# hcherkaoui/pybold

Measured on AMD Instinct MI355X. Metric: voxel-iterations/sec, higher is better.
Workload: dtype f16x2-split operands (22 bit), f32 accumulate, f64 iterate

## Files before the change

### include/pybold_hip.h

```cpp
#ifndef PYBOLD_HIP_H
#define PYBOLD_HIP_H

#include <stdint.h>

#ifdef __cplusplus
extern "C" {
#endif

#define PB_OK 0
#define PB_ERR_INVALID (-1)
#define PB_ERR_HIP (-2)

#define PB_FLAG_FORCE_GENERIC 1u
#define PB_FLAG_FORCE_FAST 2u
#define PB_FLAG_NO_PAIR 4u
#define PB_FLAG_FORCE_PAIR 8u
#define PB_FLAG_FORCE_WIDE 16u
#define PB_FLAG_DIRECT_FIR 64u
#define PB_FLAG_ONE_STREAM 128u
#define PB_FLAG_COLD_START 256u
#define PB_FLAG_NO_CERT 512u
#define PB_FLAG_CERT_NO_RESOLVE 2048u
#define PB_FLAG_FORCE_MFMA 16384u
#define PB_FLAG_NO_RHO_GUARD 32768u
#define PB_FLAG_FORCE_MFMA2 65536u
#define PB_FLAG_NO_MFMA 8192u
#define PB_FLAG_FORCE_CERT 1024u
#define PB_FLAG_NO_PARTITION 4096u
#define PB_FLAG_ONLY_DENSE 131072u
#define PB_FLAG_ONLY_SPARSE 262144u
#define PB_FLAG_NO_ILL_GUARD 524288u
#define PB_FLAG_PP_SPLIT 1048576u
#define PB_FLAG_LONG_HRF 2097152u
#define PB_FLAG_ONE_LAUNCH 32u

#define PB_STOP_NONE 0
#define PB_STOP_LOOPS 1
#define PB_STOP_WINDOW 2

int pb_version(void);

int pb_init(void);

const char* pb_last_error(void);

int pb_fista_has_fast_path(int N, int K);

int pb_fista_which_kernel(int N, int K, int P, int with_cost_trace, int stop_mode, int wind);

int pb_fista_plan(int N, int K, int P, int stop_mode, int wind, int* n_main, int* main_form,
                  int* tail_form);
int pb_fista_plan_ex(int N, int K, int P, int stop_mode, int wind, unsigned flags, int* n_main,
                     int* main_form, int* tail_form);

int pb_fista_solve(const float* y_dev, int64_t ldy, int y_rep,
                   double* w_dev, int64_t ldw, int P, int N,
                   const double* taps_host, const double* taps_dev, int K,
                   double step, double lbda, const double* lbda_dev,
                   const double* betas_dev, int n_iter,
                   float* J_dev, int64_t ldj,
                   int stop_mode, double tol, int wind, int32_t* n_done_dev,
                   unsigned flags, void* stream);

int64_t pb_fista_work_len(int P, int y_rep);
#define PB_CAND_COUNT 10
int pb_fista_list_plan(int kind, int n, int n_max, int has_pair, int has_wide, int one_stream, int has_mfma2,
                       int beside_chunks, int32_t* ranges, int32_t* bounds);
int pb_fista_solve_ex(const float* y_dev, int64_t ldy, int y_rep,
                      double* w_dev, int64_t ldw, int P, int N,
                      const double* taps_host, const double* taps_dev, int K,
                      double step, double lbda, const double* lbda_dev,
                      const double* betas_dev, int n_iter,
                      float* J_dev, int64_t ldj,
                      int stop_mode, double tol, int wind, int32_t* n_done_dev,
                      unsigned flags, void* stream,
                      const double* lmax_dev, double dense_ratio, int32_t* work_dev, int64_t work_len);

#define PB_PATH_DENSE_RATIO 0.19
#define PB_PATH_DENSE_RATIO_LONG 0.22
#define PB_PATH_DENSE_RATIO_LONGER 0.26
int64_t pb_fista_path_work_len(int P);
int pb_fista_solve_path(const float* y_dev, int64_t ldy, int y_rep, double* w_dev, int64_t ldw, int P, int N,
                        const double* taps_host, const double* taps_dev, int K, double step,
                        const double* lbda_dev, const double* lmax_dev, double dense_ratio,
                        const double* betas_dev, int n_iter, int32_t* n_done_dev, int32_t* work_dev,
                        int64_t work_len, unsigned flags, void* stream);

int pb_fista_outputs(const double* w_dev, int64_t ldw, int P, int N,
                     const double* taps_dev, int K,
                     double* z_dev, int64_t ldz, double* x_dev, int64_t ldx,
                     void* stream);

int pb_fista_stats(const double* w_dev, int64_t ldw, const float* y_dev, int64_t ldy,
                   int y_rep, int P, int N, const double* taps_dev, int K,
                   double* r2_dev, double* l1_dev, void* stream);

int pb_integ_op(const double* x_dev, int64_t ldx, double* out_dev, int64_t ldo,
                int V, int N, void* stream);
int pb_integ_adj(const double* x_dev, int64_t ldx, double* out_dev, int64_t ldo,
                 int V, int N, void* stream);
// ... 172 lines not shown
```

### pybold_amd/_lib.py

```python
import ctypes
import os

_HERE = os.path.dirname(os.path.abspath(__file__))
LIB_PATH = os.environ.get("PYBOLD_HIP_LIB") or os.path.join(_HERE, "libpybold_hip.so")

PB_FLAG_FORCE_GENERIC = 1
PB_FLAG_FORCE_FAST = 2
PB_FLAG_NO_PAIR = 4
PB_FLAG_FORCE_PAIR = 8
PB_FLAG_FORCE_WIDE = 16
PB_FLAG_ONE_LAUNCH = 32
PB_FLAG_DIRECT_FIR = 64
PB_FLAG_ONE_STREAM = 128
PB_FLAG_COLD_START = 256
PB_FLAG_NO_CERT = 512
PB_FLAG_FORCE_CERT = 1024
PB_FLAG_CERT_NO_RESOLVE = 2048
PB_FLAG_NO_PARTITION = 4096
PB_FLAG_NO_MFMA = 8192
PB_FLAG_FORCE_MFMA = 16384
PB_FLAG_NO_RHO_GUARD = 32768
PB_FLAG_FORCE_MFMA2 = 65536
PB_FLAG_ONLY_DENSE = 131072
PB_FLAG_ONLY_SPARSE = 262144
PB_FLAG_NO_ILL_GUARD = 524288
PB_FLAG_PP_SPLIT = 1048576
PB_FLAG_LONG_HRF = 2097152
PB_PATH_DENSE_RATIO = 0.19
PB_STOP_NONE = 0
PB_STOP_LOOPS = 1
PB_STOP_WINDOW = 2

_c_int = ctypes.c_int
_c_i64 = ctypes.c_int64
_c_dbl = ctypes.c_double
_ptr = ctypes.c_void_p

SIGNATURES = {
    "pb_version": (_c_int, []),
    "pb_init": (_c_int, []),
    "pb_last_error": (ctypes.c_char_p, []),
    "pb_fista_has_fast_path": (_c_int, [_c_int, _c_int]),
    "pb_fista_which_kernel": (_c_int, [_c_int, _c_int, _c_int, _c_int, _c_int, _c_int]),
    "pb_fista_plan": (_c_int, [_c_int, _c_int, _c_int, _c_int, _c_int, _ptr, _ptr, _ptr]),
    "pb_fista_plan_ex": (_c_int, [_c_int, _c_int, _c_int, _c_int, _c_int, ctypes.c_uint, _ptr, _ptr, _ptr]),
    "pb_fista_solve": (_c_int, [
        _ptr, _c_i64, _c_int,
        _ptr, _c_i64, _c_int, _c_int,
        _ptr, _ptr, _c_int,
        _c_dbl, _c_dbl, _ptr,
        _ptr, _c_int,
        _ptr, _c_i64,
        _c_int, _c_dbl, _c_int, _ptr,
        ctypes.c_uint, _ptr]),
    "pb_fista_work_len": (_c_i64, [_c_int, _c_int]),
    "pb_fista_list_plan": (_c_int, [_c_int, _c_int, _c_int, _c_int, _c_int, _c_int, _c_int, _c_int, _ptr, _ptr]),
    "pb_fista_solve_ex": (_c_int, [
        _ptr, _c_i64, _c_int,
        _ptr, _c_i64, _c_int, _c_int,
        _ptr, _ptr, _c_int,
        _c_dbl, _c_dbl, _ptr,
        _ptr, _c_int,
        _ptr, _c_i64,
        _c_int, _c_dbl, _c_int, _ptr,
        ctypes.c_uint, _ptr,
        _ptr, _c_dbl, _ptr, _c_i64]),
    "pb_fista_solve_backtrack_d": (_c_int, [
        _ptr, _c_i64, _c_int, _ptr, _c_i64, _c_int, _c_int,
        _ptr, _c_int, _c_dbl, _c_dbl, _c_int,
        _c_dbl, _ptr, _ptr, _c_int,
        _ptr, _ptr, _ptr, ctypes.c_uint, _ptr]),
    "pb_fista_path_work_len": (_c_i64, [_c_int]),
    "pb_fista_solve_path": (_c_int, [
        _ptr, _c_i64, _c_int,
        _ptr, _c_i64, _c_int, _c_int,
        _ptr, _ptr, _c_int,
        _c_dbl, _ptr, _ptr, _c_dbl,
        _ptr, _c_int,
        _ptr, _ptr, _c_i64,
        ctypes.c_uint, _ptr]),
    "pb_fista_outputs": (_c_int, [_ptr, _c_i64, _c_int, _c_int, _ptr, _c_int,
                                  _ptr, _c_i64, _ptr, _c_i64, _ptr]),
    "pb_fista_stats": (_c_int, [_ptr, _c_i64, _ptr, _c_i64, _c_int, _c_int, _c_int, _ptr,
                                _c_int, _ptr, _ptr, _ptr]),
    "pb_integ_op": (_c_int, [_ptr, _c_i64, _ptr, _c_i64, _c_int, _c_int, _ptr]),
    "pb_integ_adj": (_c_int, [_ptr, _c_i64, _ptr, _c_i64, _c_int, _c_int, _ptr]),
    "pb_conv": (_c_int, [_ptr, _c_i64, _ptr, _c_i64, _c_int, _c_int, _c_int,
                         _ptr, _c_int, _ptr]),
    "pb_corr": (_c_int, [_ptr, _c_i64, _ptr, _c_i64, _c_int, _c_int, _c_int,
# ... 181 lines not shown
```

### pybold_amd/csrc/capi.hip

```cpp
#include "../../include/pybold_hip.h"

#include <cstdarg>
#include <cstdlib>
#include <cstdio>
#include <cmath>
#include <cstring>
#include <map>
#include <mutex>

#include "fista_fast.h"
#include "generic.h"
#include "launch_fast.h"
#include "fista_pair.h"
#include "fista_pair_ffa.h"
#include "fista_exact.h"
#include "fista_exact_split.h"
#include "fista_auto.h"
#include "fista_exact_pp.h"
#include "fista_exact_split_pp.h"
#include "blind.h"
#include "fista_mfma.h"
#include "fista_mfma2.h"
#include "fista_mfma4.h"
#include "path.h"
#include "dispatch.h"

namespace {

thread_local char g_err[512] = "";

int fail(int code, const char* fmt, ...) {
  va_list ap;
  va_start(ap, fmt);
  vsnprintf(g_err, sizeof(g_err), fmt, ap);
  va_end(ap);
  return code;
}

int check_launch(const char* what) {
  hipError_t e = hipGetLastError();
  if (e != hipSuccess) return fail(PB_ERR_HIP, "%s: %s", what, hipGetErrorString(e));
  g_err[0] = 0;
  return PB_OK;
}

constexpr int LDS_DOUBLES_MAX = 20000;
inline int64_t gen_lds_doubles(int N, int K, int stop_mode, int wind) {
  return 3 * (int64_t)N + K + 2 * pb::GEN_WAVES + (stop_mode == PB_STOP_WINDOW ? (int64_t)wind * N : 0);
}

constexpr int AUTO_LAUNCH_ITERS = 65536, AUTO_RESIDENT_WAVES = 2048;
inline int auto_outer_chunk(int V, int nb_sub_iter) {
  const int64_t rounds = ((int64_t)V + AUTO_RESIDENT_WAVES - 1) / AUTO_RESIDENT_WAVES;
  const int64_t per = (int64_t)(nb_sub_iter > 0 ? nb_sub_iter : 1) * (rounds > 0 ? rounds : 1);
// ... 648 lines not shown
    return run_partition(r, a, lf, user, taps_host, taps_dev, flags, dense_ratio, work_dev);
  if (r.path != PATH_GENERIC) return run_in_place(r, a, lf, user, flags);
  if (flags & PB_FLAG_FORCE_FAST)
    return fail(PB_ERR_INVALID, "pb_fista_solve: no register-resident kernel for N=%d K=%d stop=%d",
                N, K, stop_mode);
  if (!taps_dev) return fail(PB_ERR_INVALID, "pb_fista_solve: taps_dev required for the generic kernel");
  if (gen_lds_doubles(N, K, stop_mode, wind) > LDS_DOUBLES_MAX)
    return fail(PB_ERR_INVALID, "pb_fista_solve: N=%d K=%d wind=%d exceeds LDS", N, K, wind);
  launch_generic(a, taps_dev, K, wind, J_dev != nullptr, false, P, user);
  return check_launch("fista_generic_kernel");
}

int pb_fista_list_plan(int kind, int n, int n_max, int has_pair, int has_wide, int one_stream, int has_mfma2,
                       int beside_chunks, int32_t* ranges, int32_t* bounds) {
  if (kind < 1 || kind > 3 || n < 0 || n_max < n) return fail(PB_ERR_INVALID, "pb_fista_list_plan: bad argument");
  Piece pc[pb::MAX_PIECES];
  int npc = 0;
  const double slots = wave_slots();
  if (n > 0 && kind == 1) npc = pb::plan_pieces_mfma(n, has_pair != 0, has_wide != 0, false, one_stream != 0, has_mfma2 != 0, beside_chunks, slots, pc);
  else if (n > 0 && kind == 2) npc = pb::plan_pieces(n, has_pair != 0, has_wide != 0, false, one_stream != 0, slots, pc);
  else if (kind == 3 && n_max > 0)
    npc = pb::plan_partitioned(n, n_max, has_pair != 0, has_wide != 0, one_stream != 0, has_mfma2 != 0, beside_chunks, slots, pc);
  int32_t rg[2 * pb::CAND_COUNT];
  const int rc = pb::plan_to_candidates(pc, npc, rg);
  for (int c = 0; c < pb::CAND_COUNT; ++c) {
    if (ranges) { ranges[2 * c] = rg[2 * c]; ranges[2 * c + 1] = rg[2 * c + 1]; }
    if (bounds) bounds[c] = pb::cand_max_slots(c, n_max, slots);
  }
  if (rc != 0) return fail(PB_ERR_INVALID, "pb_fista_list_plan: a piece of the plan found its candidate launch taken (n=%d)", n);
  g_err[0] = 0;
  return PB_OK;
}

int64_t pb_fista_work_len(int P, int y_rep) {
  if (P < 0 || y_rep < 1) return 0;
  return work_layout(P, (P + y_rep - 1) / y_rep).total;
}

int pb_fista_solve_ex(const float* y_dev, int64_t ldy, int y_rep, double* w_dev, int64_t ldw, int P,
                      int N, const double* taps_host, const double* taps_dev, int K, double step,
                      double lbda, const double* lbda_dev, const double* betas_dev, int n_iter, float* J_dev,
                      int64_t ldj, int stop_mode, double tol, int wind, int32_t* n_done_dev,
                      unsigned flags, void* stream, const double* lmax_dev, double dense_ratio,
                      int32_t* work_dev, int64_t work_len) {
  return solve_impl(y_dev, ldy, y_rep, w_dev, ldw, P, N, taps_host, taps_dev, K, step, lbda, lbda_dev, betas_dev, n_iter,
                    J_dev, ldj, stop_mode, tol, wind, n_done_dev, flags, stream, lmax_dev, dense_ratio, work_dev, work_len);
}

int pb_fista_solve(const float* y_dev, int64_t ldy, int y_rep, double* w_dev, int64_t ldw, int P,
                   int N, const double* taps_host, const double* taps_dev, int K, double step,
                   double lbda,
                   const double* lbda_dev, const double* betas_dev, int n_iter, float* J_dev,
                   int64_t ldj, int stop_mode, double tol, int wind, int32_t* n_done_dev,
                   unsigned flags, void* stream) {
  int32_t* work = nullptr;
  int64_t len = 0;
  if (P >= PART_MIN_P && N <= 1280 && n_done_dev && !(flags & PB_FLAG_NO_PARTITION) && !stream_is_capturing((hipStream_t)stream))
    work = own_workspace(stream, work_layout(P, (P + (y_rep > 0 ? y_rep : 1) - 1) / (y_rep > 0 ? y_rep : 1)).total, &len);
  return solve_impl(y_dev, ldy, y_rep, w_dev, ldw, P, N, taps_host, taps_dev, K, step, lbda, lbda_dev, betas_dev, n_iter,
                    J_dev, ldj, stop_mode, tol, wind, n_done_dev, flags, stream, nullptr, 0.0, work, len);
}

namespace {
int long_hrf_entry(const char* name, int N, int K, int stop_mode, int wind, unsigned flags, const ExactLongEntry** le) {
  if (flags & (PB_FLAG_FORCE_GENERIC | PB_FLAG_FORCE_FAST | PB_FLAG_PP_SPLIT))
    return fail(PB_ERR_INVALID, "%s: PB_FLAG_LONG_HRF names the 48-tap register form; it excludes PB_FLAG_FORCE_GENERIC, PB_FLAG_FORCE_FAST and PB_FLAG_PP_SPLIT", name);
// ... 763 lines not shown
```

### pybold_amd/csrc/dispatch.h

```cpp
#pragma once
#include "../../include/pybold_hip.h"
#include "fista_fast.h"
#include "launch_fast.h"
#include "fista_pair.h"
#include "fista_pair_ffa.h"
#include "fista_exact.h"
#include "fista_exact_split.h"
#include "fista_auto.h"
#include "fista_auto_split.h"
#include "fista_exact_pp.h"
#include "fista_exact_long.h"
#include "fista_exact_split_long.h"
#include "fista_mfma.h"
#include "fista_mfma2.h"
#include "fista_mfma4.h"
#include "path.h"

namespace {

typedef int (*fast_launch_fn)(const pb::FistaArgs&, const double* taps, int K, bool with_j,
                              int stop, hipStream_t);
typedef int (*fast_launch_pp_fn)(const pb::FistaArgs&, int stop, hipStream_t);
typedef int (*launch_fn)(const pb::FistaArgs&, const double* taps, int K, bool with_j, hipStream_t);
typedef int (*pair_cert_fn)(const pb::FistaArgs&, const double* taps, int K, hipStream_t);
typedef int (*pair_split_fn)(const pb::FistaArgs&, const double* taps, int K, bool with_j, bool cert, hipStream_t);

struct FastEntry {
  int S, KT;
  fast_launch_fn fn;
  fast_launch_pp_fn fn_pp;
  launch_fn fn_pair;
  launch_fn fn_pair_ffa;
  int (*fn_pair_dev)(const pb::FistaArgs&, hipStream_t);
  pair_cert_fn fn_pair_cert;
  pair_split_fn fn_pair_split;
};

}

namespace pb {
#define PB_FAST(S, KT)                                                                              \
  extern template int launch_fast<S, KT>(const FistaArgs&, const double*, int, bool, int, hipStream_t); \
  extern template int launch_fast_pp<S, KT>(const FistaArgs&, int, hipStream_t);            \
  extern template int launch_pair<S, KT>(const FistaArgs&, const double*, int, bool, hipStream_t); \
  extern template int launch_pair_ffa<S, KT>(const FistaArgs&, const double*, int, bool, hipStream_t); \
  extern template int launch_pair_ffa_dev<S, KT>(const FistaArgs&, hipStream_t);                  \
  extern template int launch_pair_ffa_cert<S, KT>(const FistaArgs&, const double*, int, hipStream_t); \
  extern template int launch_pair_ffa_split<S, KT>(const FistaArgs&, const double*, int, bool, bool, hipStream_t);
#include "fast_table.inc"
#undef PB_FAST
}

namespace pb {
#define PB_MFMA(NB) extern template int launch_mfma<NB>(const FistaArgs&, const double*, int, bool, hipStream_t);
PB_MFMA(5) PB_MFMA(6) PB_MFMA(7) PB_MFMA(8) PB_MFMA(9) PB_MFMA(10)
#undef PB_MFMA
}
namespace pb {
#define PB_MFMA2(A, B) extern template int launch_mfma2<A, B>(const FistaArgs&, const double*, int, bool, hipStream_t);
PB_MFMA2(2, 3) PB_MFMA2(3, 3) PB_MFMA2(3, 4) PB_MFMA2(4, 4) PB_MFMA2(4, 5) PB_MFMA2(5, 5) PB_MFMA2(5, 6) PB_MFMA2(6, 6)
PB_MFMA2(6, 7) PB_MFMA2(7, 7) PB_MFMA2(7, 8) PB_MFMA2(8, 8) PB_MFMA2(8, 9) PB_MFMA2(9, 9) PB_MFMA2(9, 10) PB_MFMA2(10, 10)
#undef PB_MFMA2
#define PB_MFMA4(A) extern template int launch_mfma4<A>(const FistaArgs&, const double*, int, bool, hipStream_t);
PB_MFMA4(6) PB_MFMA4(7) PB_MFMA4(8) PB_MFMA4(9) PB_MFMA4(10)
#undef PB_MFMA4
}
namespace {
launch_fn pick_mfma2(int N, int K, bool two_tiles_only) {
  static const launch_fn tab[] = {
      &pb::launch_mfma2<2, 3>, &pb::launch_mfma2<3, 3>, &pb::launch_mfma2<3, 4>, &pb::launch_mfma2<4, 4>,
      &pb::launch_mfma2<4, 5>, &pb::launch_mfma2<5, 5>, &pb::launch_mfma2<5, 6>, &pb::launch_mfma2<6, 6>,
      &pb::launch_mfma2<6, 7>, &pb::launch_mfma2<7, 7>, &pb::launch_mfma2<7, 8>, &pb::launch_mfma2<8, 8>,
      &pb::launch_mfma2<8, 9>, &pb::launch_mfma2<9, 9>, &pb::launch_mfma2<9, 10>, &pb::launch_mfma2<10, 10>};
  const int nb = (N + 31) / 32;
  if (K < 1 || K > 65 || nb < 5 || nb > 20) return nullptr;
  if (K > 33 && (two_tiles_only || N <= 224)) return nullptr;
  return tab[nb - 5];
}
launch_fn pick_mfma4(int N, int K, bool two_tiles_only) {
  static const launch_fn tab[] = {&pb::launch_mfma4<6>, &pb::launch_mfma4<7>, &pb::launch_mfma4<8>, &pb::launch_mfma4<9>,
                                  &pb::launch_mfma4<10>};
  if (K < 1 || K > 65 || (K > 33 && two_tiles_only) || N <= 640 || N > 1280) return nullptr;
  return tab[(N + 127) / 128 - 6];
}
constexpr int MFMA_K2 = 33, MFMA_K3 = 64;
constexpr int MFMA1_NMAX = 10 * pb::MFMA_SPAN;
launch_fn pick_mfma(int N, int K, bool stop_rule) {
  static const launch_fn tab[] = {&pb::launch_mfma<5>, &pb::launch_mfma<6>, &pb::launch_mfma<7>,
                                  &pb::launch_mfma<8>, &pb::launch_mfma<9>, &pb::launch_mfma<10>};
  const int nb = (N + pb::MFMA_SPAN - 1) / pb::MFMA_SPAN;
  if (K < 1 || K > MFMA_K3 || (K > MFMA_K2 && stop_rule) || N <= 128 || nb > 10) return nullptr;
  return tab[nb - 5];
}
}
namespace pb {
#define PB_WIDE(S, KT)                                                                            \
  extern template int launch_wide<S, KT>(const FistaArgs&, const double*, int, bool, int, hipStream_t); \
  extern template int launch_wide_pp<S, KT>(const FistaArgs&, int, hipStream_t);
#include "wide_table.inc"
#undef PB_WIDE
}
namespace {

typedef int (*wide_launch_fn)(const pb::FistaArgs&, const double* taps, int K, bool with_j, int stop,
                              hipStream_t);
struct WideEntry {
  int S, KT;
  wide_launch_fn fn;
  fast_launch_pp_fn fn_pp;
};
#define PB_WIDE(S, KT) {S, KT, &pb::launch_wide<S, KT>, &pb::launch_wide_pp<S, KT>},
const WideEntry kWide[] = {
#include "wide_table.inc"
};
#undef PB_WIDE

template <class Entry, size_t n>
const Entry* pick_cheapest(const Entry (&tab)[n], int N, int K, int per_lane) {
  const Entry* best = nullptr;
  const int s_need = (N + per_lane - 1) / per_lane;
  for (const Entry& e : tab) {
    if (e.S < s_need || e.KT < K) continue;
    if (!best || (int64_t)e.S * e.KT < (int64_t)best->S * best->KT) best = &e;
  }
  return best;
// ... 347 lines not shown
    r.cert = split_pair_cert;
    r.has_pair = r.se && (plain || split_pair_cert);
    return r;
  }
  const bool forced = (fl & PB_FLAG_FORCE_MFMA2) != 0;
  const bool forced_short = c.reported && forced && (plain || window6) && pick_mfma2(N, K, true);
  const launch_fn split = mfma4 ? mfma4 : ((mfma2 && ((forced && (!c.reported || long_shape || forced_short)) || long_call)) ? mfma2 : nullptr);
  if (split && (backup_ok || forced_short)) {
    r.path = PATH_SPLIT_LONG;
    r.split = split;
    r.fe = fe1;
    r.we = we1;
    const bool one_launch = (fl & PB_FLAG_ONE_LAUNCH) != 0;
    r.base = (fl & PB_FLAG_FORCE_MFMA2) ? P : (mfma4 ? mfma4_base(P, one_launch) : mfma2_long_base(P, one_launch));
    return r;
  }
  const bool mfma_plain = plain && c.n_done && (!c.lbda_vec || (fl & PB_FLAG_FORCE_MFMA)) && !(fl & FLAGS_VECTOR_ONLY) &&
                          mfma_serves_plain(N, K);
  if (!mfma_plain && !(fl & FLAGS_NO_SPLIT_PAIR) && r.se && (P >= SPLIT_MIN_P || (fl & PB_FLAG_FORCE_PAIR)) &&
      (plain || split_pair_cert)) {
    r.path = PATH_SPLIT_PAIR;
    r.we = we1;
    r.cert = split_pair_cert;
    return r;
  }
  const FastEntry* fe = (fl & (PB_FLAG_FORCE_GENERIC | PB_FLAG_FORCE_WIDE)) ? nullptr : fe1;
  if (fe && !ring_fits(fe->S, stop, c.wind)) fe = nullptr;
  if (fe) {
    r.fe = fe;
    r.cert = window6 && fe->fn_pair_cert && c.n_done && (P >= 2 || c.reported) && !(fl & (PB_FLAG_NO_PAIR | PB_FLAG_DIRECT_FIR)) &&
             cert_clears(CERT_TN_VECTOR);
    r.mfma_cert = r.cert && ((fl & PB_FLAG_FORCE_MFMA) || c.tol_iters < CERT_TN_MATRIX_PIPE);
    const bool mfma_rule = plain || r.mfma_cert || (stop == PB_STOP_LOOPS && !c.cost_trace && K <= MFMA_K2);
    const launch_fn mfma_shape = mfma_rule ? pick_mfma(N, K, !plain) : nullptr;
    const launch_fn mfma = (mfma_shape && c.n_done && (!c.lbda_vec || (fl & PB_FLAG_FORCE_MFMA)) && !(fl & FLAGS_PAIR_PIN_OR_NO_MFMA))
                               ? mfma_shape : nullptr;
    r.has_pair = (fe->fn_pair && plain) || r.cert;
    r.we = pick_wide_small(N, K);
    r.has_wide = r.we != nullptr;
    r.beside_chunks = beside_chunks_for(N);
    r.path = PATH_PIECES;
    if (fl & PB_FLAG_NO_PAIR) {
      r.one_form = FORM_FAST1;
      return r;
    }
    const bool part_mfma = mfma || (c.lbda_vec && mfma_shape);
    if (part_ws && (part_mfma || !(fl & PB_FLAG_NO_ILL_GUARD))) {
      r.path = PATH_PART_SHORT;
      r.mfma = part_mfma ? mfma_shape : nullptr;
      r.split = !part_mfma ? nullptr
                : (mfma2 || !c.lbda_vec) ? mfma2
                : ((plain || split_cert) && K <= MFMA_K2) ? pick_mfma2(N, K, false) : nullptr;
      r.has_mfma2 = r.split && (plain || r.mfma_cert);
      return r;
    }
    r.mfma = mfma;
    r.split = mfma2;
    r.has_mfma2 = c.reported ? (plain || window6) && pick_mfma2(N, K, true) : mfma2 && (plain || r.mfma_cert);
    if (fl & PB_FLAG_FORCE_PAIR) r.one_form = (r.cert || (fe->fn_pair && P >= 2 && plain)) ? FORM_PAIR : FORM_FAST1;
    return r;
  }
  const launch_fn mf = mfma_plain ? pick_mfma(N, K, false) : nullptr;
  if (mf && we1) {
    r.path = PATH_MFMA_WIDE;
    r.mfma = mf;
    r.we = we1;
    r.base = mfma_wide_base(P, (fl & PB_FLAG_ONE_LAUNCH) != 0);
    return r;
  }
  if (!(fl & PB_FLAG_FORCE_GENERIC) && we1 && ring_fits(we1->S, stop, c.wind)) {
    r.path = PATH_WIDE;
    r.we = we1;
    return r;
  }
  r.path = PATH_GENERIC;
  return r;
}

Route route_pp(int N, int K, int P, bool shared, int stop_mode, bool n_done, unsigned fl) {
  Route r{};
  const bool plain_shared = shared && stop_mode == PB_STOP_NONE;
  const WideEntry* we1 = pick_wide(N, K);
  if (N > MFMA1_NMAX && plain_shared && n_done && K <= 65 && !(fl & FLAGS_VECTOR_ONLY)) {
    const bool four = N > 640;
    const launch_fn split = four ? pick_mfma4(N, K, false) : pick_mfma2(N, K, false);
    if (split && we1 && (four || P >= mfma2_long_min_p(K) || (fl & PB_FLAG_FORCE_MFMA2))) {
      const bool all = (fl & (PB_FLAG_ONE_LAUNCH | PB_FLAG_FORCE_MFMA2)) != 0;
      r.path = PATH_SPLIT_LONG;
      r.split = split;
      r.we = we1;
      r.backup_wide = true;
      r.base = four ? mfma4_base(P, all) : mfma2_long_base(P, all);
      return r;
    }
  }
  r.fe = (fl & PB_FLAG_FORCE_GENERIC) ? nullptr : pick_fast(N, K);
  if (r.fe) {
    r.path = PATH_PIECES;
    r.one_stream = true;
    r.we = pick_wide_small(N, K);
    r.has_wide = r.we != nullptr;
    if (plain_shared && r.fe->fn_pair_dev && P >= 2 && !(fl & (PB_FLAG_NO_PAIR | PB_FLAG_DIRECT_FIR))) {
      r.has_pair = true;
      r.beside_chunks = MFMA2_BESIDE_CHUNKS;
      if (fl & PB_FLAG_FORCE_PAIR) {
        r.one_form = FORM_PAIR;
        return r;
      }
      r.mfma = (n_done && !(fl & PB_FLAG_NO_MFMA)) ? pick_mfma(N, K, false) : nullptr;
      r.split = (r.mfma && K <= MFMA_K2) ? pick_mfma2(N, K, false) : nullptr;
      r.has_mfma2 = r.split != nullptr;
      return r;
    }
    const bool wide_first = r.we && !(fl & (PB_FLAG_NO_PAIR | PB_FLAG_FORCE_PAIR | PB_FLAG_ONE_LAUNCH)) && best_form(P, false, true) == FORM_WIDE;
    r.one_form = wide_first ? FORM_WIDE : FORM_FAST1;
    return r;
  }
  r.we = (fl & PB_FLAG_FORCE_GENERIC) ? nullptr : we1;
  r.path = r.we ? PATH_WIDE : PATH_GENERIC;
  return r;
}

int route_pieces(const Route& r, int P, bool one_launch, bool one_stream, Piece* pc) {
  if (r.one_form) {
    pc[0] = Piece{r.one_form, 0, P, false, false};
    return 1;
  }
  if (r.mfma) return plan_pieces_mfma(P, r.has_pair, r.has_wide, one_launch, one_stream, r.has_mfma2, r.beside_chunks, pc);
  return plan_pieces(P, r.has_pair, r.has_wide, one_launch, one_stream, pc);
}

void report(const Route& r, int N, int P, bool one_launch, bool one_stream, int* nm, int* mf, int* tf) {
  auto passes = [&](int base, int form, int rest) {
    if (base > 0 && base < P) { *nm = base; *mf = form; *tf = rest; }
    else *tf = base > 0 ? form : rest;
  };
  *nm = *mf = *tf = 0;
  switch (r.path) {
    case PATH_SPLIT_LONG: passes(r.base, N > 640 ? pb::FORM_MFMA4 : FORM_MFMA2, r.backup_wide ? FORM_WIDE : FORM_FAST1); return;
    case PATH_MFMA_WIDE: passes(r.base, FORM_MFMA, FORM_WIDE); return;
    case PATH_SPLIT_PAIR: *tf = FORM_PAIR; return;
    case PATH_WIDE: *tf = FORM_WIDE; return;
// ... 20 lines not shown
```

### pybold_amd/solver.py

```python
import numpy as np
import torch

from . import _lib
from ._lib import (PB_FLAG_COLD_START, PB_FLAG_NO_CERT, PB_FLAG_FORCE_CERT, PB_FLAG_DIRECT_FIR, PB_FLAG_ONE_STREAM, PB_FLAG_FORCE_FAST, PB_FLAG_FORCE_GENERIC, PB_FLAG_FORCE_PAIR, PB_FLAG_FORCE_WIDE,
                   PB_FLAG_NO_PAIR, PB_FLAG_ONE_LAUNCH, PB_STOP_LOOPS, PB_STOP_NONE, PB_STOP_WINDOW)

_STOP = {None: PB_STOP_NONE, "none": PB_STOP_NONE, "loops": PB_STOP_LOOPS,
         "window": PB_STOP_WINDOW}
_FORCE = {None: 0, "generic": PB_FLAG_FORCE_GENERIC, "fast": PB_FLAG_FORCE_FAST,
          "fast1": PB_FLAG_FORCE_FAST | PB_FLAG_NO_PAIR | PB_FLAG_ONE_LAUNCH,
          "fast2": PB_FLAG_FORCE_FAST | PB_FLAG_FORCE_PAIR | PB_FLAG_ONE_LAUNCH,
          "fast2d": PB_FLAG_FORCE_FAST | PB_FLAG_FORCE_PAIR | PB_FLAG_ONE_LAUNCH | PB_FLAG_DIRECT_FIR,
          "direct": PB_FLAG_DIRECT_FIR,
          "wide": PB_FLAG_FORCE_FAST | PB_FLAG_FORCE_WIDE | PB_FLAG_ONE_LAUNCH,
          "one": PB_FLAG_ONE_LAUNCH, "seq": PB_FLAG_ONE_STREAM,
          "cert": PB_FLAG_FORCE_CERT, "cert2": PB_FLAG_FORCE_CERT | PB_FLAG_FORCE_PAIR | PB_FLAG_ONE_LAUNCH,
          "certonly": PB_FLAG_FORCE_CERT | PB_FLAG_FORCE_PAIR | PB_FLAG_ONE_LAUNCH | _lib.PB_FLAG_CERT_NO_RESOLVE,
          "nocert": PB_FLAG_NO_CERT,
          "valu": _lib.PB_FLAG_NO_MFMA, "valuseq": _lib.PB_FLAG_NO_MFMA | PB_FLAG_ONE_STREAM,
          "mfma": PB_FLAG_ONE_LAUNCH | _lib.PB_FLAG_FORCE_MFMA,
          "path_dense": _lib.PB_FLAG_ONLY_DENSE, "path_sparse": _lib.PB_FLAG_ONLY_SPARSE,
          "noill": _lib.PB_FLAG_NO_ILL_GUARD,
          "nopart": _lib.PB_FLAG_NO_PARTITION, "nopartseq": _lib.PB_FLAG_NO_PARTITION | PB_FLAG_ONE_STREAM,
          "mfma2": _lib.PB_FLAG_FORCE_MFMA2, "mfma2only": _lib.PB_FLAG_FORCE_MFMA2 | _lib.PB_FLAG_CERT_NO_RESOLVE,
          "mfma2cert": _lib.PB_FLAG_FORCE_MFMA2 | PB_FLAG_FORCE_CERT,
          "mfma2certonly": _lib.PB_FLAG_FORCE_MFMA2 | PB_FLAG_FORCE_CERT | _lib.PB_FLAG_CERT_NO_RESOLVE,
          "intermediate": _lib.PB_FLAG_NO_RHO_GUARD,
          "intermediate_noresolve": _lib.PB_FLAG_NO_RHO_GUARD | _lib.PB_FLAG_CERT_NO_RESOLVE,
          "noresolve": _lib.PB_FLAG_CERT_NO_RESOLVE,
          "mfmaonly": PB_FLAG_ONE_LAUNCH | _lib.PB_FLAG_FORCE_MFMA | _lib.PB_FLAG_CERT_NO_RESOLVE,
          "mfmacert": PB_FLAG_ONE_LAUNCH | _lib.PB_FLAG_FORCE_MFMA | PB_FLAG_FORCE_CERT,
          "mfmacertonly": PB_FLAG_ONE_LAUNCH | _lib.PB_FLAG_FORCE_MFMA | PB_FLAG_FORCE_CERT | _lib.PB_FLAG_CERT_NO_RESOLVE}


_warned = set()


def warn_once(key, message):
    if key not in _warned:
        _warned.add(key)
        import warnings
        warnings.warn(message, RuntimeWarning, stacklevel=3)


def _warn_if_slow_kernel(lib, N, K, P, want_J, stop, wind, flags):
    if P < 256 or (flags & (PB_FLAG_FORCE_GENERIC | PB_FLAG_FORCE_FAST)):
        return
    form = lib.pb_fista_which_kernel(int(N), int(K), int(P), int(bool(want_J)), _STOP[stop], int(wind))
    if form in (1, 2, 3) and P >= 16384 and not (flags & (_lib.PB_FLAG_NO_MFMA | PB_FLAG_NO_PAIR | PB_FLAG_FORCE_PAIR | PB_FLAG_FORCE_WIDE)):
        why = []
        if N <= 128:
            why = []
        elif N > 1280:
# ... 983 lines not shown
```

Baseline: 4.712 billion.

## Use 2:4 sparse SMFMAC tiles for MFMA FISTA convolution when K ≤ 32

```diff
diff --git a/include/pybold_hip.h b/include/pybold_hip.h
--- a/include/pybold_hip.h
+++ b/include/pybold_hip.h
@@ -32,6 +32,7 @@
 #define PB_FLAG_NO_ILL_GUARD 524288u
 #define PB_FLAG_PP_SPLIT 1048576u
 #define PB_FLAG_LONG_HRF 2097152u
+enum { PB_FLAG_MFMA_DENSE_TILES = 4194304 };
 #define PB_FLAG_ONE_LAUNCH 32u
 
 #define PB_STOP_NONE 0
@@ -66,6 +67,8 @@
 #define PB_CAND_COUNT 10
 int pb_fista_list_plan(int kind, int n, int n_max, int has_pair, int has_wide, int one_stream, int has_mfma2,
                        int beside_chunks, int32_t* ranges, int32_t* bounds);
+int pb_mfma_sparse_tile(const double* taps_host, int K, int pass, int parity, int row_half, unsigned short* hi,
+                        unsigned short* lo, unsigned short* idx, float* c64);
 int pb_fista_solve_ex(const float* y_dev, int64_t ldy, int y_rep,
                       double* w_dev, int64_t ldw, int P, int N,
                       const double* taps_host, const double* taps_dev, int K,
diff --git a/pybold_amd/_lib.py b/pybold_amd/_lib.py
--- a/pybold_amd/_lib.py
+++ b/pybold_amd/_lib.py
@@ -25,6 +25,7 @@
 PB_FLAG_ONLY_SPARSE = 262144
 PB_FLAG_NO_ILL_GUARD = 524288
 PB_FLAG_PP_SPLIT = 1048576
+PB_FLAG_MFMA_DENSE_TILES = 4194304
 PB_FLAG_LONG_HRF = 2097152
 PB_PATH_DENSE_RATIO = 0.19
 PB_STOP_NONE = 0
@@ -55,6 +56,7 @@
         ctypes.c_uint, _ptr]),
     "pb_fista_work_len": (_c_i64, [_c_int, _c_int]),
     "pb_fista_list_plan": (_c_int, [_c_int, _c_int, _c_int, _c_int, _c_int, _c_int, _c_int, _c_int, _ptr, _ptr]),
+    "pb_mfma_sparse_tile": (_c_int, [_ptr, _c_int, _c_int, _c_int, _c_int, _ptr, _ptr, _ptr, _ptr]),
     "pb_fista_solve_ex": (_c_int, [
         _ptr, _c_i64, _c_int,
         _ptr, _c_i64, _c_int, _c_int,
diff --git a/pybold_amd/csrc/capi.hip b/pybold_amd/csrc/capi.hip
--- a/pybold_amd/csrc/capi.hip
+++ b/pybold_amd/csrc/capi.hip
@@ -20,6 +20,7 @@
 #include "fista_exact_split_pp.h"
 #include "blind.h"
 #include "fista_mfma.h"
+#include "fista_mfma_sparse.h"
 #include "fista_mfma2.h"
 #include "fista_mfma4.h"
 #include "path.h"
@@ -734,6 +735,22 @@
   return PB_OK;
 }
 
+int pb_mfma_sparse_tile(const double* taps_host, int K, int pass, int parity, int row_half, unsigned short* hi,
+                        unsigned short* lo, unsigned short* idx, float* c64) {
+  if (!taps_host || !hi || !lo || !idx) return fail(PB_ERR_INVALID, "pb_mfma_sparse_tile: NULL pointer");
+  if (pass < 0 || pass > 1 || parity < 0 || parity > 1 || row_half < 0 || row_half > 1)
+    return fail(PB_ERR_INVALID, "pb_mfma_sparse_tile: pass, parity and row_half are 0 or 1");
+  if (K < 1 || K > pb::SPARSE_TILE_KMAX)
+    return fail(PB_ERR_INVALID, "pb_mfma_sparse_tile: K=%d outside 1..%d taps (33 taps put three nonzeros in a group of four)", K,
+                pb::SPARSE_TILE_KMAX);
+  const pb::MfmaTaps tp = pb::make_mfma_taps(taps_host, K);
+  if (pb::build_sparse_tile_host(tp, K, pass, parity, row_half, hi, lo, idx) != 0)
+    return fail(PB_ERR_INVALID, "pb_mfma_sparse_tile: a group of four holds more than two nonzeros (K=%d)", K);
+  if (c64) memcpy(c64, tp.c, 64 * sizeof(float));
+  g_err[0] = 0;
+  return PB_OK;
+}
+
 int64_t pb_fista_work_len(int P, int y_rep) {
   if (P < 0 || y_rep < 1) return 0;
   return work_layout(P, (P + y_rep - 1) / y_rep).total;
diff --git a/pybold_amd/csrc/dispatch.h b/pybold_amd/csrc/dispatch.h
--- a/pybold_amd/csrc/dispatch.h
+++ b/pybold_amd/csrc/dispatch.h
@@ -55,6 +55,9 @@
 #define PB_MFMA(NB) extern template int launch_mfma<NB>(const FistaArgs&, const double*, int, bool, hipStream_t);
 PB_MFMA(5) PB_MFMA(6) PB_MFMA(7) PB_MFMA(8) PB_MFMA(9) PB_MFMA(10)
 #undef PB_MFMA
+#define PB_MFMA(NB) extern template int launch_mfma_st<NB>(const FistaArgs&, const double*, int, bool, hipStream_t);
+PB_MFMA(5) PB_MFMA(6) PB_MFMA(7) PB_MFMA(8) PB_MFMA(9) PB_MFMA(10)
+#undef PB_MFMA
 }
 namespace pb {
 #define PB_MFMA2(A, B) extern template int launch_mfma2<A, B>(const FistaArgs&, const double*, int, bool, hipStream_t);
@@ -85,12 +88,14 @@
 }
 constexpr int MFMA_K2 = 33, MFMA_K3 = 64;
 constexpr int MFMA1_NMAX = 10 * pb::MFMA_SPAN;
-launch_fn pick_mfma(int N, int K, bool stop_rule) {
+launch_fn pick_mfma(int N, int K, bool stop_rule, bool dense_tiles = false) {
   static const launch_fn tab[] = {&pb::launch_mfma<5>, &pb::launch_mfma<6>, &pb::launch_mfma<7>,
                                   &pb::launch_mfma<8>, &pb::launch_mfma<9>, &pb::launch_mfma<10>};
+  static const launch_fn tab_st[] = {&pb::launch_mfma_st<5>, &pb::launch_mfma_st<6>, &pb::launch_mfma_st<7>,
+                                     &pb::launch_mfma_st<8>, &pb::launch_mfma_st<9>, &pb::launch_mfma_st<10>};
   const int nb = (N + pb::MFMA_SPAN - 1) / pb::MFMA_SPAN;
   if (K < 1 || K > MFMA_K3 || (K > MFMA_K2 && stop_rule) || N <= 128 || nb > 10) return nullptr;
-  return tab[nb - 5];
+  return (dense_tiles ? tab : tab_st)[nb - 5];
 }
 }
 namespace pb {
@@ -504,7 +509,7 @@
              cert_clears(CERT_TN_VECTOR);
     r.mfma_cert = r.cert && ((fl & PB_FLAG_FORCE_MFMA) || c.tol_iters < CERT_TN_MATRIX_PIPE);
     const bool mfma_rule = plain || r.mfma_cert || (stop == PB_STOP_LOOPS && !c.cost_trace && K <= MFMA_K2);
-    const launch_fn mfma_shape = mfma_rule ? pick_mfma(N, K, !plain) : nullptr;
+    const launch_fn mfma_shape = mfma_rule ? pick_mfma(N, K, !plain, (fl & PB_FLAG_MFMA_DENSE_TILES) != 0) : nullptr;
     const launch_fn mfma = (mfma_shape && c.n_done && (!c.lbda_vec || (fl & PB_FLAG_FORCE_MFMA)) && !(fl & FLAGS_PAIR_PIN_OR_NO_MFMA))
                                ? mfma_shape : nullptr;
     r.has_pair = (fe->fn_pair && plain) || r.cert;
@@ -532,7 +537,7 @@
     if (fl & PB_FLAG_FORCE_PAIR) r.one_form = (r.cert || (fe->fn_pair && P >= 2 && plain)) ? FORM_PAIR : FORM_FAST1;
     return r;
   }
-  const launch_fn mf = mfma_plain ? pick_mfma(N, K, false) : nullptr;
+  const launch_fn mf = mfma_plain ? pick_mfma(N, K, false, (fl & PB_FLAG_MFMA_DENSE_TILES) != 0) : nullptr;
   if (mf && we1) {
     r.path = PATH_MFMA_WIDE;
     r.mfma = mf;
@@ -579,7 +584,7 @@
         r.one_form = FORM_PAIR;
         return r;
       }
-      r.mfma = (n_done && !(fl & PB_FLAG_NO_MFMA)) ? pick_mfma(N, K, false) : nullptr;
+      r.mfma = (n_done && !(fl & PB_FLAG_NO_MFMA)) ? pick_mfma(N, K, false, (fl & PB_FLAG_MFMA_DENSE_TILES) != 0) : nullptr;
       r.split = (r.mfma && K <= MFMA_K2) ? pick_mfma2(N, K, false) : nullptr;
       r.has_mfma2 = r.split != nullptr;
       return r;
diff --git a/pybold_amd/csrc/fista_mfma_sparse.h b/pybold_amd/csrc/fista_mfma_sparse.h
--- /dev/null
+++ b/pybold_amd/csrc/fista_mfma_sparse.h
@@ -0,0 +1,337 @@
+#pragma once
+#include "fista_mfma.h"
+#include "mfma_sparse_tiles.h"
+
+namespace pb {
+
+typedef _Float16 h16 __attribute__((ext_vector_type(16)));
+typedef unsigned u8 __attribute__((ext_vector_type(8)));
+
+__device__ __forceinline__ f4 smfmac_part(const Frag& A, int idx, const u8& bh, const u8& bl, f4 acc, int part) {
+  return part == 0   ? __builtin_amdgcn_smfmac_f32_16x16x64_f16(A.hi, __builtin_bit_cast(h16, bh), acc, idx, 0, 0)
+         : part == 1 ? __builtin_amdgcn_smfmac_f32_16x16x64_f16(A.hi, __builtin_bit_cast(h16, bl), acc, idx, 0, 0)
+                     : __builtin_amdgcn_smfmac_f32_16x16x64_f16(A.lo, __builtin_bit_cast(h16, bh), acc, idx, 0, 0);
+}
+
+template <int NB, bool TAPS_DEV = false>
+__global__ __launch_bounds__(256) void fista_mfma_sparse_kernel(FistaArgs a, MfmaTaps tp) {
+  const int lane = threadIdx.x & 63;
+  const int v = lane & 15, g = lane >> 4;
+  const int wave = (int)((blockIdx.x * 256 + threadIdx.x) >> 6);
+  int s0, n_list;
+  launch_slots(a, s0, n_list);
+  if (__builtin_amdgcn_readfirstlane(wave) * 16 + s0 >= n_list) return;
+  bool live;
+  const int p = slot_to_problem(a, wave * 16 + v + s0, n_list, live);
+  const int tb = 8 * g;
+  const bool g3 = g == 3;
+
+  extern __shared__ __attribute__((aligned(16))) char mf_smem[];
+  u4* lrf = reinterpret_cast<u4*>(mf_smem) + ((threadIdx.x >> 6) * NB * 2 * 64 + lane);
+  float* lc = reinterpret_cast<float*>(mf_smem + (size_t)4 * NB * 2 * 64 * sizeof(u4)) + (threadIdx.x >> 6) * 64;
+  double step = a.step, g_scale = tp.g_scale;
+  float y_scale = tp.y_scale;
+  if constexpr (TAPS_DEV) {
+    double run = 0.0;
+    for (int k = 0; k <= lane && k < a.K; ++k) run += (double)(float)a.taps_pp[k];
+    float cm = fabsf((float)run);
+#pragma unroll
+    for (int o = 1; o < 64; o <<= 1) cm = fmaxf(cm, __shfl_xor(cm, o, 64));
+    int e = 0;
+    if (cm > 0.0f) (void)frexpf(cm, &e);
+    const int sa = 3 - e;
+    lc[lane] = (float)ldexp(run, sa);
+    g_scale = ldexp(1.0, -2 * sa);
+    y_scale = ldexpf(1.0f, sa);
+    step = a.step_vec[0];
+  } else {
+    lc[lane] = tp.c[lane];
+  }
+  wave_sync();
+
+  Frag At[2][2][2];
+  int ai[2][2][2];
+  {
+    auto cval = [&](int lag) -> float { return lag < 0 ? 0.0f : lc[lag > 63 ? 63 : lag]; };
+#pragma unroll
+    for (int ps = 0; ps < 2; ++ps)
+#pragma unroll
+      for (int par = 0; par < 2; ++par)
+#pragma unroll
+        for (int r = 0; r < 2; ++r) {
+          float val[8];
+          unsigned ix;
+          (void)sparse_tile_lane(cval, ps, par, r, lane, val, ix);
+          At[ps][par][r] = split8(val);
+          ai[ps][par][r] = (int)ix;
+        }
+  }
+
+  const double lb = a.lbda_vec ? a.lbda_vec[p] : a.lbda;
+  float ysn[NB][8];
+  double w[NB][8];
+  float sigma = 1.0f, inv_sigma = 1.0f;
+  bool degenerate = false;
+  {
+    const float* yrow = a.y + (int64_t)(p / a.y_rep) * a.ldy;
+    float m = 0.0f;
+#pragma unroll
+    for (int q = 0; q < NB; ++q)
+#pragma unroll
+      for (int j = 0; j < 8; ++j) {
+        const int t = MFMA_SPAN * q + tb + j;
+        float yv;
+        if (q == NB - 1) {
+          const bool ok = t < a.N && !(j == 7 && g3);
+          float yl = yrow[t < a.N ? t : a.N - 1];
+          asm volatile("" : "+v"(yl));
+          yv = ok ? yl : 0.0f;
+        } else if (j == 7) {
+          float yl = yrow[t];
+          asm volatile("" : "+v"(yl));
+          yv = g3 ? 0.0f : yl;
+        } else {
+          yv = yrow[t];
+        }
+        ysn[q][j] = yv;
+        m = fmaxf(m, fabsf(yv));
+      }
+    m = group_max(m);
+    {
+      const bool okm = m > 0.0f && m < 3.0e38f;
+      int e = 0;
+      (void)frexpf(okm ? m : 1.0f, &e);
+      const float sg = ldexpf(1.0f, a.ybits - e) / y_scale, isg = ldexpf(1.0f, e - a.ybits) * y_scale;
+      sigma = okm ? sg : 1.0f;
+      inv_sigma = okm ? isg : 1.0f;
+      degenerate = !okm && !a.cold;
+    }
+    const float ys = -sigma * y_scale;
+    const double* wrow = a.w + (int64_t)p * a.ldw;
+#pragma unroll
+    for (int q = 0; q < NB; ++q)
+#pragma unroll
+      for (int j = 0; j < 8; ++j) {
+        ysn[q][j] *= ys;
+        w[q][j] = 0.0;
+      }
+    if (!a.cold) {
+#pragma unroll
+      for (int q = 0; q < NB; ++q)
+#pragma unroll
+        for (int j = 0; j < 8; ++j) {
+          const int t = MFMA_SPAN * q + tb + j;
+          if (q == NB - 1) {
+            double wl = wrow[t < a.N ? t : a.N - 1] * (double)sigma;
+            asm volatile("" : "+v"(wl));
+            w[q][j] = (t < a.N && !(j == 7 && g3)) ? wl : 0.0;
+          } else if (j == 7) {
+            double wl = wrow[t] * (double)sigma;
+            asm volatile("" : "+v"(wl));
+            w[q][j] = g3 ? 0.0 : wl;
+          } else {
+            w[q][j] = wrow[t] * (double)sigma;
+          }
+        }
+    }
+  }
+  const double th = lb * step * (double)sigma;
+  const double nstep = -step * g_scale;
+  const double nstep7 = g3 ? 0.0 : nstep;
+  float guard = 0.0f, wlast = 0.0f;
+  double unused0 = 0.0, unused1 = 0.0;
+
+#pragma unroll
+  for (int ps = 0; ps < 2; ++ps)
+#pragma unroll
+    for (int par = 0; par < 2; ++par)
+#pragma unroll
+      for (int r = 0; r < 2; ++r) asm volatile("" : "+a"(At[ps][par][r].hi), "+a"(At[ps][par][r].lo));
+#pragma unroll
+  for (int q = 0; q < NB; ++q)
+#pragma unroll
+    for (int j = 0; j < 8; ++j) asm volatile("" : "+a"(ysn[q][j]));
+
+  u8 rth, rtl;
+  auto forward = [&]() __attribute__((always_inline)) {
+    u8 bh, bl;
+    f4 acc[NB][2];
+    float xf[NB][8];
+    unsigned rh[NB][4], rl[NB][4];
+    float remf = 0.0f;
+    auto cvt_pair = [&](auto qc, auto pc) {
+      constexpr int q = decltype(qc)::value, pp = decltype(pc)::value;
+      float x0, x1;
+      const double w0 = w[q][2 * pp], w1 = w[q][2 * pp + 1];
+      asm volatile("v_cvt_f32_f64 %0, %1" : "=v"(x0) : "v"(w0));
+      asm volatile("v_cvt_f32_f64 %0, %1" : "=v"(x1) : "v"(w1));
+      xf[q][2 * pp] = x0;
+      xf[q][2 * pp + 1] = x1;
+    };
+    auto split_block = [&](auto qc, auto pc) {
+      constexpr int q = decltype(qc)::value, pp = decltype(pc)::value;
+      float x0 = xf[q][2 * pp], x1 = xf[q][2 * pp + 1];
+      if constexpr (pp == 3 && q >= 1) {
+        const float d = acc[q - 1][1][3] + remf;
+        x1 = g3 ? d : x1;
+      }
+      unsigned h2, l2;
+      if constexpr (PB_MFMA_REM && pp == 3 && q + 1 < NB) split_pair_rem(x0, x1, h2, l2, remf);
+      else split_pair(x0, x1, h2, l2);
+      bh[2 * pp + (q & 1)] = h2;
+      bl[2 * pp + (q & 1)] = l2;
+    };
+    auto cinit = [&](auto qc, auto rc) {
+      constexpr int q = decltype(qc)::value, r = decltype(rc)::value;
+      acc[q][r] = f4{ysn[q][4 * r + 0], ysn[q][4 * r + 1], ysn[q][4 * r + 2], ysn[q][4 * r + 3]};
+    };
+    auto finish_pair = [&](auto qc, auto pc) {
+      constexpr int q = decltype(qc)::value, pp = decltype(pc)::value;
+      float x0 = acc[q][pp >> 1][(2 * pp) & 3], x1 = acc[q][pp >> 1][(2 * pp + 1) & 3];
+      if constexpr (q == NB - 1) {
+        x0 = (MFMA_SPAN * q + tb + 2 * pp < a.N) ? x0 : 0.0f;
+        x1 = (MFMA_SPAN * q + tb + 2 * pp + 1 < a.N && !(pp == 3 && g3)) ? x1 : 0.0f;
+      }
+      split_pair(x0, x1, rh[q][pp], rl[q][pp]);
+      if constexpr (q == NB - 1) {
+        rth[2 * pp + (q & 1)] = rh[q][pp];
+        rtl[2 * pp + (q & 1)] = rl[q][pp];
+        rth[2 * pp + 1 - (q & 1)] = 0u;
+        rtl[2 * pp + 1 - (q & 1)] = 0u;
+      }
+      if constexpr (pp == 3) {
+        lrf[(2 * q) * 64] = u4{rh[q][0], rh[q][1], rh[q][2], rh[q][3]};
+        lrf[(2 * q + 1) * 64] = u4{rl[q][0], rl[q][1], rl[q][2], rl[q][3]};
+      }
+    };
+    static_for<0, 4>([&](auto pc) {
+      constexpr int pp = decltype(pc)::value;
+      cvt_pair(std::integral_constant<int, 0>{}, pc);
+      bh[2 * pp + 1] = 0u;
+      bl[2 * pp + 1] = 0u;
+    });
+    static_for<0, 4>([&](auto pc) { split_block(std::integral_constant<int, 0>{}, pc); });
+    cinit(std::integral_constant<int, 0>{}, std::integral_constant<int, 0>{});
+    cinit(std::integral_constant<int, 0>{}, std::integral_constant<int, 1>{});
+    static_for<0, NB>([&](auto qc) {
+      constexpr int q = decltype(qc)::value;
+      static_for<0, 6>([&](auto sc) {
+        constexpr int sl = decltype(sc)::value;
+        constexpr int r = (sl == 1 || sl >= 4) ? 0 : 1, part = sl < 2 ? 0 : (sl == 2 || sl == 4 ? 1 : 2);
+        acc[q][r] = smfmac_part(At[0][q & 1][r], ai[0][q & 1][r], bh, bl, acc[q][r], part);
+        if constexpr (sl < 4) {
+          if constexpr (q >= 1) finish_pair(std::integral_constant<int, q - 1>{}, sc);
+          if constexpr (q + 1 < NB) cvt_pair(std::integral_constant<int, q + 1>{}, sc);
+        } else {
+          if constexpr (q + 1 < NB) cinit(std::integral_constant<int, q + 1>{}, std::integral_constant<int, sl - 4>{});
+        }
+      });
+      __builtin_amdgcn_sched_barrier(0);
+      if constexpr (q + 1 < NB) static_for<0, 4>([&](auto pc) { split_block(std::integral_constant<int, q + 1>{}, pc); });
+    });
+    static_for<0, 4>([&](auto pc) { finish_pair(std::integral_constant<int, NB - 1>{}, pc); });
+  };
+  auto backward = [&](const double beta) __attribute__((always_inline)) {
+    const double nb1 = -(1.0 + beta);
+    f4 acc[NB][2];
+    unsigned fh3[NB], fl3[NB];
+    float remb = 0.0f;
+    const unsigned psel = g3 ? 0x07060100u : 0x03020100u;
+    auto fetch = [&](auto qc) {
+      constexpr int q = decltype(qc)::value;
+      typedef const volatile __attribute__((address_space(3))) unsigned lds_word;
+      lds_word* ph3 = (lds_word*)reinterpret_cast<const unsigned*>(&lrf[(2 * q) * 64]);
+      lds_word* pl3 = (lds_word*)reinterpret_cast<const unsigned*>(&lrf[(2 * q + 1) * 64]);
+#pragma unroll
+      for (int c = 0; c < 3; ++c) {
+        rth[2 * c + (q & 1)] = ph3[c];
+        rtl[2 * c + (q & 1)] = pl3[c];
+      }
+      fh3[q] = ph3[3];
+      fl3[q] = pl3[3];
+    };
+    auto patch = [&](auto qc) {
+      constexpr int q = decltype(qc)::value;
+      const float d = acc[q + 1][1][3] + remb;
+      const unsigned h2 = __builtin_bit_cast(unsigned, __builtin_amdgcn_cvt_pkrtz(d, d));
+      float l;
+      asm("v_fma_mix_f32 %0, %1, -1.0, %2 op_sel_hi:[1,0,0]" : "=v"(l) : "v"(h2), "v"(d));
+      const unsigned l2 = pk_rne(l, l);
+      if constexpr (PB_MFMA_REM && q >= 1) asm("v_fma_mix_f32 %0, %1, -1.0, %2 op_sel_hi:[1,0,0]" : "=v"(remb) : "v"(l2), "v"(l));
+      rth[6 + (q & 1)] = __builtin_amdgcn_perm(h2, fh3[q], psel);
+      rtl[6 + (q & 1)] = __builtin_amdgcn_perm(l2, fl3[q], psel);
+    };
+    auto update = [&](auto qc, auto jc) {
+      constexpr int q = decltype(qc)::value, j = decltype(jc)::value;
+      (void)fista_update<false>(w[q][j], acc[q][j >> 2][j & 3], j == 7 ? nstep7 : nstep, th, nb1, unused0, unused1);
+    };
+    static_for<0, NB>([&](auto qq) {
+      constexpr int q = NB - 1 - decltype(qq)::value;
+      static_for<0, 6>([&](auto sc) {
+        constexpr int sl = decltype(sc)::value;
+        constexpr int r = (sl == 1 || sl >= 4) ? 0 : 1, part = sl < 2 ? 0 : (sl == 2 || sl == 4 ? 1 : 2);
+        if constexpr (part == 0) acc[q][r] = smfmac_part(At[1][q & 1][r], ai[1][q & 1][r], rth, rtl, f4{0.f, 0.f, 0.f, 0.f}, 0);
+        else acc[q][r] = smfmac_part(At[1][q & 1][r], ai[1][q & 1][r], rth, rtl, acc[q][r], part);
+        if constexpr (sl >= 1 && sl < 5) {
+          if constexpr (q + 1 < NB) update(std::integral_constant<int, q + 1>{}, std::integral_constant<int, sl - 1>{});
+        }
+      });
+      __builtin_amdgcn_sched_barrier(0);
+      if constexpr (q >= 1) fetch(std::integral_constant<int, q - 1>{});
+      if constexpr (q + 1 < NB) static_for<4, 8>([&](auto jc) { update(std::integral_constant<int, q + 1>{}, jc); });
+      if constexpr (q >= 1) patch(std::integral_constant<int, q - 1>{});
+    });
+    static_for<0, 8>([&](auto jc) { update(std::integral_constant<int, 0>{}, jc); });
+  };
+  auto range_check = [&]() {
+    const float m = iterate_absmax<NB>(w);
+    wlast = m;
+    guard = __builtin_fmaxf(guard, __builtin_fmaxf(m, residual_guard<NB>(lrf)));
+  };
+
+  for (int it = 0; it < a.n_iter; ++it) {
+    const double beta = a.betas[it];
+    forward();
+    backward(beta);
+    if (PB_MFMA_CHECKS && (((it & 7) == 7) || (it == a.n_iter - 1) || (it == 0 && !a.cold))) range_check();
+  }
+
+  guard = group_max(guard);
+  wlast = group_max(wlast);
+  const bool bad = !(guard < 60000.0f) || degenerate || (a.rho_guard && wlast > 0.0f && (float)th > MFMA_RHO_MAX * wlast);
+  if (live && !bad) {
+    double* wrow = a.w + (int64_t)p * a.ldw;
+#pragma unroll
+    for (int q = 0; q < NB; ++q)
+#pragma unroll
+      for (int j = 0; j < 8; ++j) {
+        const int t = MFMA_SPAN * q + tb + j;
+        if (t < a.N && !(j == 7 && g3)) wrow[t] = w[q][j] * (double)inv_sigma;
+      }
+  }
+  if (live && a.n_done && g == 0) a.n_done[p] = bad ? -1 : a.n_iter;
+}
+
+template <int NB>
+int launch_mfma_sparse(const FistaArgs& a, const double* taps, int K, hipStream_t st) {
+  if (K < 1 || K > SPARSE_TILE_KMAX || a.N > MFMA_SPAN * NB || a.N <= MFMA_SPAN * (NB - 1)) return 1;
+  const int64_t waves = (launch_count(a) + 15) / 16;
+  const dim3 grid((unsigned)((waves + 3) / 4)), block(256);
+  const size_t lds = (size_t)4 * NB * 2 * 64 * sizeof(u4) + 4 * 64 * sizeof(float);
+  if (a.taps_pp) {
+    const MfmaTaps none{};
+    hipLaunchKernelGGL((fista_mfma_sparse_kernel<NB, true>), grid, block, lds, st, a, none);
+    return 0;
+  }
+  const MfmaTaps tp = make_mfma_taps(taps, K);
+  hipLaunchKernelGGL((fista_mfma_sparse_kernel<NB, false>), grid, block, lds, st, a, tp);
+  return 0;
+}
+
+template <int NB>
+int launch_mfma_st(const FistaArgs& a, const double* taps, int K, bool with_j, hipStream_t st) {
+  if (K <= SPARSE_TILE_KMAX && !with_j && a.stop_mode == PB_STOP_NONE) return launch_mfma_sparse<NB>(a, taps, K, st);
+  return launch_mfma<NB>(a, taps, K, with_j, st);
+}
+
+}
diff --git a/pybold_amd/csrc/mfma_sparse_inst.hip b/pybold_amd/csrc/mfma_sparse_inst.hip
--- /dev/null
+++ b/pybold_amd/csrc/mfma_sparse_inst.hip
@@ -0,0 +1,8 @@
+#include "fista_mfma_sparse.h"
+#ifndef PB_NB
+#error "compile with -DPB_NB=<blocks of 31 samples>"
+#endif
+namespace pb {
+extern template int launch_mfma<PB_NB>(const FistaArgs&, const double*, int, bool, hipStream_t);
+template int launch_mfma_st<PB_NB>(const FistaArgs&, const double*, int, bool, hipStream_t);
+}
diff --git a/pybold_amd/csrc/mfma_sparse_tiles.h b/pybold_amd/csrc/mfma_sparse_tiles.h
--- /dev/null
+++ b/pybold_amd/csrc/mfma_sparse_tiles.h
@@ -0,0 +1,77 @@
+#pragma once
+#include "mfma_core.h"
+
+namespace pb {
+
+constexpr int SPARSE_TILE_KMAX = 32;
+
+template <typename CV>
+__host__ __device__ __forceinline__ float sparse_tile_entry(CV&& cval, int pass, bool own, int ko, int ki) {
+  const float S = cval(63);
+  const int d = pass == 0 ? ko - ki : ki - ko;
+  if (own) {
+    if (ko == 31) return ki == 31 ? 1.0f : 1.0f / (float)(1 << 9);
+    if (ki == 31) return S * (float)(1 << 9);
+    return cval(d);
+  }
+  if (ko == 31 || ki == 31) return 0.0f;
+  return cval(31 + d) - S;
+}
+
+template <typename CV>
+__host__ __device__ __forceinline__ bool sparse_tile_lane(CV&& cval, int pass, int par, int r, int lane, float (&val)[8], unsigned& idx) {
+  const int rho = lane & 15, kg = lane >> 4, ko = 8 * (rho >> 2) + 4 * r + (rho & 3);
+  bool ok = true;
+  idx = 0;
+#pragma unroll
+  for (int p = 0; p < 4; ++p) {
+    const int gb = 2 * (kg & 1) + (p >> 1), t = 2 * (kg >> 1) + (p & 1);
+    float d[4];
+#pragma unroll
+    for (int pos = 0; pos < 4; ++pos) d[pos] = sparse_tile_entry(cval, pass, (pos >> 1) == par, ko, 8 * gb + 2 * t + (pos & 1));
+    const bool n0 = d[0] != 0.0f, n1 = d[1] != 0.0f, n2 = d[2] != 0.0f, n3 = d[3] != 0.0f;
+    ok = ok && ((int)n0 + (int)n1 + (int)n2 + (int)n3 <= 2);
+    int i0 = n0 ? 0 : (n1 ? 1 : (n2 ? 2 : 3));
+    int i1 = n3 ? 3 : (n2 ? 2 : (n1 ? 1 : 0));
+    if (i0 >= i1) {
+      const bool none = !(n0 || n1 || n2 || n3);
+      const int z = i0;
+      i0 = none ? 0 : (z < 3 ? z : 2);
+      i1 = none ? 1 : (z < 3 ? z + 1 : 3);
+    }
+    val[2 * p] = i0 == 0 ? d[0] : (i0 == 1 ? d[1] : d[2]);
+    val[2 * p + 1] = i1 == 1 ? d[1] : (i1 == 2 ? d[2] : d[3]);
+    idx |= (unsigned)(i0 | (i1 << 2)) << (4 * p);
+  }
+  return ok;
+}
+
+inline unsigned short host_f16_bits(_Float16 h) { return __builtin_bit_cast(unsigned short, h); }
+inline _Float16 host_f16_rtz(float x) {
+  _Float16 h = (_Float16)x;
+  if (fabsf((float)h) > fabsf(x)) {
+    h = __builtin_bit_cast(_Float16, (unsigned short)(host_f16_bits(h) - 1));
+  }
+  return h;
+}
+
+inline int build_sparse_tile_host(const MfmaTaps& tp, int K, int pass, int par, int r, unsigned short* hi, unsigned short* lo, unsigned short* idx) {
+  if (K < 1 || K > SPARSE_TILE_KMAX) return 1;
+  auto cval = [&](int lag) -> float { return lag < 0 ? 0.0f : tp.c[lag > 63 ? 63 : lag]; };
+  for (int lane = 0; lane < 64; ++lane) {
+    float val[8];
+    unsigned ix;
+    if (!sparse_tile_lane(cval, pass, par, r, lane, val, ix)) return 1;
+    const int rho = lane & 15, kg = lane >> 4;
+    for (int j = 0; j < 8; ++j) {
+      const _Float16 h = host_f16_rtz(val[j]);
+      const _Float16 l = (_Float16)(val[j] - (float)h);
+      hi[rho * 32 + 8 * kg + j] = host_f16_bits(h);
+      lo[rho * 32 + 8 * kg + j] = host_f16_bits(l);
+    }
+    idx[rho * 4 + kg] = (unsigned short)ix;
+  }
+  return 0;
+}
+
+}
diff --git a/pybold_amd/solver.py b/pybold_amd/solver.py
--- a/pybold_amd/solver.py
+++ b/pybold_amd/solver.py
@@ -19,6 +19,9 @@
           "nocert": PB_FLAG_NO_CERT,
           "valu": _lib.PB_FLAG_NO_MFMA, "valuseq": _lib.PB_FLAG_NO_MFMA | PB_FLAG_ONE_STREAM,
           "mfma": PB_FLAG_ONE_LAUNCH | _lib.PB_FLAG_FORCE_MFMA,
+          "mfma_dense": PB_FLAG_ONE_LAUNCH | _lib.PB_FLAG_FORCE_MFMA | _lib.PB_FLAG_MFMA_DENSE_TILES,
+          "dense_tiles": _lib.PB_FLAG_MFMA_DENSE_TILES,
+          "mfma_denseonly": PB_FLAG_ONE_LAUNCH | _lib.PB_FLAG_FORCE_MFMA | _lib.PB_FLAG_MFMA_DENSE_TILES | _lib.PB_FLAG_CERT_NO_RESOLVE,
           "path_dense": _lib.PB_FLAG_ONLY_DENSE, "path_sparse": _lib.PB_FLAG_ONLY_SPARSE,
           "noill": _lib.PB_FLAG_NO_ILL_GUARD,
           "nopart": _lib.PB_FLAG_NO_PARTITION, "nopartseq": _lib.PB_FLAG_NO_PARTITION | PB_FLAG_ONE_STREAM,
```

After: 4.857 billion (median of 6 runs). +3.1%, better.
